# Audio-WestlakeU/FullSubNet

Measured on AMD Instinct MI355X. Metric: frames/sec (16 kHz, 512-FFT, hop 256), whole job, higher is better.
Workload: dtype f32

## Files before the change

### fullsubnet_amd/csrc/lstm_rec_x_kernels.hip

```cpp
#include "fsn_common.h"
#include "lstm_cell.h"

namespace {

__device__ __forceinline__ void lds_dma_fragment(const float* g, unsigned lds_base) {
    unsigned saved;
    asm volatile(
        "s_mov_b32 %0, m0\n\t"
        "s_mov_b32 m0, %1\n\t"
        "s_nop 0\n\t"
        "global_load_lds_dwordx4 %2, off\n\t"
        "s_nop 0\n\t"
        "s_mov_b32 m0, %0"
        : "=&s"(saved)
        : "s"(lds_base), "v"(g)
        : "memory");
}

__device__ __forceinline__ void lds_dma_fragment_s(const float* sbase, unsigned lane_bytes, unsigned lds_base) {
    unsigned saved;
    asm volatile(
        "s_mov_b32 %0, m0\n\t"
        "s_mov_b32 m0, %1\n\t"
        "s_nop 0\n\t"
        "global_load_lds_dwordx4 %2, %3\n\t"
        "s_nop 0\n\t"
        "s_mov_b32 m0, %0"
        : "=&s"(saved)
        : "s"(lds_base), "v"(lane_bytes), "s"(sbase)
        : "memory");
}

#ifndef FSN_REC_VCAP
#define FSN_REC_VCAP 76
#endif
template <int H, int RT, int UG, bool GRU, bool HSEQ>
__global__ __launch_bounds__((H / (16 * UG)) * 64) __attribute__((amdgpu_num_vgpr(FSN_REC_VCAP))) void lstm_rec_x_kernel(const float* __restrict__ xseq,
                                                                          const float* __restrict__ w_p,
                                                                          unsigned whh_off,
                                                                          const float* __restrict__ bias, int Tp,
                                                                          int Npad, const FsnRecFc fc) {
    constexpr int NW = H / (16 * UG);
    constexpr int KC = H / 16;
    constexpr int HS = H + 4;
    constexpr int ROWS = RT * 16;
    constexpr int SK = 6;
    constexpr int NSL = KC / SK;
    constexpr int NF = RT * SK;
    static_assert(KC % SK == 0 && SK % 2 == 0 && KC % 2 == 0, "slice width must divide the K range; chunks go in pairs");
    extern __shared__ __attribute__((aligned(16))) float xs[];
    float* hl = xs + 2 * NF * 256;
    float* wl = hl + ROWS * HS;

    const int lane = threadIdx.x & 63, wave = __builtin_amdgcn_readfirstlane(threadIdx.x >> 6);
    const int lr = lane & 15, lq = lane >> 4;
    const long n0 = (long)blockIdx.x * ROWS;
    if (!HSEQ)
        for (int i = threadIdx.x; i < 2 * H; i += NW * 64) {
            const int c = i / H, k = i % H;
            wl[i] = fc.w_p[(((k >> 4) * 64) + ((k & 15) >> 2) * 16 + c) * 4 + (k & 3)];
        }
    int fc_b0 = 0, fc_f0 = 0;
    float fc_bias0 = 0.f, fc_bias1 = 0.f;
    if (!HSEQ) {
        const long ng0 = n0 + fc.row0;
        fc_b0 = (int)(ng0 / fc.F);
        fc_f0 = (int)(ng0 - (long)fc_b0 * fc.F);
        fc_bias0 = fc.bias[0];
        fc_bias1 = fc.bias[1];
    }
    static_assert(RT >= 2 && RT <= 4, "two base registers reach row tiles 0-1 / 2-3");
    static_assert(!GRU || NSL % 2 == 0, "the GRU form skips whole passes of the x ring: slices per pass must be even");
    f32x4 cst[RT][UG], tmp[RT][UG];
#pragma unroll
    for (int rt = 0; rt < RT; ++rt)
#pragma unroll
        for (int u = 0; u < UG; ++u)
#pragma unroll
            for (int i = 0; i < 4; ++i) cst[rt][u][i] = 0.f;
    for (int i = threadIdx.x; i < ROWS * HS; i += NW * 64) hl[i] = 0.f;

    const unsigned xlane = (unsigned)(lr * H + 4 * lq);
    const unsigned xs_lds = (unsigned)(size_t)(__attribute__((address_space(3))) float*)xs;
    auto fill = [&](int buf, int t, int sl) {
        const float* src = xseq + ((long)t * Npad + n0) * H + sl * (SK * 16);
        for (int f = wave; f < NF; f += NW) {
            const int rt = f / SK, kcl = f - rt * SK;
            lds_dma_fragment(src + (rt * 16 * H + kcl * 16) + xlane,
                             __builtin_amdgcn_readfirstlane(xs_lds + (unsigned)((buf * NF + f) * 1024)));
        }
    };
    constexpr int FPW = (NF + NW - 1) / NW;
    int fsa_src[FPW], fsa_lds[FPW];
#pragma unroll
    for (int i = 0; i < FPW; ++i) {
        const int f = wave + i * NW, rt = f / SK, kcl = f - rt * SK;
        fsa_src[i] = __builtin_amdgcn_readfirstlane(rt * 16 * H + kcl * 16);
        fsa_lds[i] = __builtin_amdgcn_readfirstlane((int)xs_lds + f * 1024);
    }
    const unsigned xlane_bytes = xlane * 4u;
    auto fill_s = [&](int buf, int t, int sl) {
        const float* src = xseq + ((long)t * Npad + n0) * H + sl * (SK * 16);
#pragma unroll
        for (int i = 0; i < FPW; ++i)
            if (NF % NW == 0 || wave + i * NW < NF)
                lds_dma_fragment_s(src + fsa_src[i], xlane_bytes, (unsigned)(fsa_lds[i] + buf * (NF * 1024)));
    };
    fill(0, 0, 0);
    asm volatile("s_waitcnt vmcnt(0)" ::: "memory");
    __syncthreads();

    f32x4 b0[UG], b1[UG];
    const __amdgpu_buffer_rsrc_t wrsrc =
        __builtin_amdgcn_make_buffer_rsrc(const_cast<float*>(w_p), 0, 0x7fffffff, 0x00020000);
    const unsigned lane16 = (unsigned)lane * 16u;
    auto wofs = [&](int g, int u) { return (unsigned)((g * KC + wave * UG + u) * KC) * 256u; };
    auto wload = [&](unsigned ofs) {
        return __builtin_bit_cast(f32x4, __builtin_amdgcn_raw_buffer_load_b128(wrsrc, lane16, ofs * 4u, 0));
    };
    float bias_n[UG];
    {
        int g0 = 1;
        asm volatile("" : "+s"(g0));
#pragma unroll
        for (int u = 0; u < UG; ++u) {
            b0[u] = wload(wofs(g0, u));
            bias_n[u] = bias[(g0 * KC + wave * UG + u) * 16 + lr];
        }
    }
    auto mma = [&](f32x4 (&acc)[RT][UG], const float* a, int a_rt_stride, const f32x4 (&b)[UG]) {
#pragma unroll
        for (int rt = 0; rt < RT; ++rt) {
            const f32x4 av = *reinterpret_cast<const f32x4*>(a + rt * a_rt_stride);
#pragma unroll
            for (int jj = 0; jj < 4; ++jj)
#pragma unroll
                for (int u = 0; u < UG; ++u) acc[rt][u] = mfma16(av[jj], b[u][jj], acc[rt][u]);
        }
    };

    auto mma_fill = [&](f32x4 (&acc)[RT][UG], const float* a, int a_rt_stride, const f32x4 (&b)[UG], int buf, int nt, int nsl) {
        const f32x4 a0 = *reinterpret_cast<const f32x4*>(a), a1 = *reinterpret_cast<const f32x4*>(a + a_rt_stride);
#pragma unroll
        for (int jj = 0; jj < 4; ++jj)
#pragma unroll
            for (int u = 0; u < UG; ++u) acc[0][u] = mfma16(a0[jj], b[u][jj], acc[0][u]);
        __builtin_amdgcn_sched_barrier(0);
        if (nt < Tp) fill_s(buf, nt, nsl);
        __builtin_amdgcn_sched_barrier(0);
#pragma unroll
        for (int rt = 1; rt < RT; ++rt) {
            const f32x4 av = rt == 1 ? a1 : *reinterpret_cast<const f32x4*>(a + rt * a_rt_stride);
#pragma unroll
            for (int jj = 0; jj < 4; ++jj)
#pragma unroll
                for (int u = 0; u < UG; ++u) acc[rt][u] = mfma16(av[jj], b[u][jj], acc[rt][u]);
        }
    };

    for (int t = 0; t < Tp; ++t) {
#pragma unroll
        for (int pass = 0; pass < 4; ++pass) {
            __builtin_amdgcn_sched_barrier(0);
            int g = pass == 0 ? 1 : (pass == 1 ? 0 : pass);
            int gn = pass == 0 ? 0 : (pass == 1 ? 2 : (pass == 2 ? 3 : 1));
            asm volatile("" : "+s"(g));
            asm volatile("" : "+s"(gn));
            const bool hpart = t > 0 && !(GRU && pass == 2);
            const bool xpart = !(GRU && pass == 1 && t > 0);
            const bool prev_h = t > 0 && !(GRU && pass == 3);
            f32x4 acc[RT][UG];
            unsigned wx[UG], wh[UG], wxn[UG];
#pragma unroll
            for (int u = 0; u < UG; ++u) {
                wx[u] = wofs(g, u);
                wh[u] = wx[u] + whh_off;
                wxn[u] = wofs(gn, u) + ((GRU && pass == 0 && t > 0) ? whh_off : 0u);
                const float b = bias_n[u];
#pragma unroll
                for (int rt = 0; rt < RT; ++rt) acc[rt][u] = f32x4{b, b, b, b};
                bias_n[u] = bias[(gn * KC + wave * UG + u) * 16 + lr];
            }
#pragma unroll 1
            for (int sl = 0; sl < (xpart ? NSL : 0); ++sl) {
                const int j = pass * NSL + sl;
                if (j > 0 && !(sl == 0 && prev_h)) {
                    asm volatile("s_waitcnt vmcnt(%0)" ::"n"(UG) : "memory");
                    __builtin_amdgcn_fence(__ATOMIC_RELEASE, "workgroup", "local");
                    __builtin_amdgcn_s_barrier();
                    __builtin_amdgcn_fence(__ATOMIC_ACQUIRE, "workgroup", "local");
                }
                const int nsl = sl + 1 < NSL ? sl + 1 : 0;
                const int nt = (sl + 1 < NSL || pass < 3) ? t : t + 1;
                const float* xa = xs + ((j & 1) * NF) * 256 + lane * 4;
#pragma unroll
                for (int kk = 0; kk < SK; kk += 2) {
                    const int kc = sl * SK + kk;
#pragma unroll
                    for (int u = 0; u < UG; ++u)
                        b1[u] = wload(wx[u] + (unsigned)(kc + 1) * 256u);
                    __builtin_amdgcn_sched_barrier(0);
                    if (kk == 0) mma_fill(acc, xa, SK * 256, b0, (j + 1) & 1, nt, nsl);
                    else mma(acc, xa + kk * 256, SK * 256, b0);
                    __builtin_amdgcn_sched_barrier(0);
                    const bool more_x = kc + 2 < KC;
#pragma unroll
                    for (int u = 0; u < UG; ++u) {
                        b0[u] = wload(more_x ? wx[u] + (unsigned)(kc + 2) * 256u : (hpart ? wh[u] : wxn[u]));
                    }
                    __builtin_amdgcn_sched_barrier(0);
                    mma(acc, xa + (kk + 1) * 256, SK * 256, b1);
                    __builtin_amdgcn_sched_barrier(0);
                }
            }
            if (hpart) {
                typedef const __attribute__((address_space(3))) float* lds_cptr;
                unsigned hb01 = (unsigned)(size_t)(lds_cptr)(hl + lr * HS + 4 * lq), hb23 = hb01 + 32u * HS * 4u;
                asm volatile("" : "+v"(hb01));
                asm volatile("" : "+v"(hb23));
                lds_cptr ha01 = (lds_cptr)(size_t)hb01;
                lds_cptr ha23 = (lds_cptr)(size_t)hb23;
                auto mmah = [&](int kofs, const f32x4 (&b)[UG]) {
#pragma unroll
                    for (int rt = 0; rt < RT; ++rt) {
                        const f32x4 av = *reinterpret_cast<const __attribute__((address_space(3))) f32x4*>((rt < 2 ? ha01 : ha23) + (rt & 1) * 16 * HS + kofs);
#pragma unroll
                        for (int jj = 0; jj < 4; ++jj)
#pragma unroll
                            for (int u = 0; u < UG; ++u) acc[rt][u] = mfma16(av[jj], b[u][jj], acc[rt][u]);
                    }
                };
#pragma unroll 1
                for (int hs = 0; hs < NSL; ++hs) {
                    if (pass < 3 && hs == NSL / 2) {
                        asm volatile("s_waitcnt vmcnt(%0)" ::"n"(UG) : "memory");
                        __builtin_amdgcn_fence(__ATOMIC_RELEASE, "workgroup", "local");
                        __builtin_amdgcn_s_barrier();
                        __builtin_amdgcn_fence(__ATOMIC_ACQUIRE, "workgroup", "local");
                    }
#pragma unroll
                    for (int kk = 0; kk < SK; kk += 2) {
                        const int kc = hs * SK + kk;
#pragma unroll
                        for (int u = 0; u < UG; ++u) b1[u] = wload(wh[u] + (unsigned)(kc + 1) * 256u);
                        __builtin_amdgcn_sched_barrier(0);
                        mmah(kk * 16, b0);
                        __builtin_amdgcn_sched_barrier(0);
                        const bool more_h = kc + 2 < KC;
#pragma unroll
                        for (int u = 0; u < UG; ++u) b0[u] = wload(more_h ? wh[u] + (unsigned)(kc + 2) * 256u : wxn[u]);
                        __builtin_amdgcn_sched_barrier(0);
                        mmah((kk + 1) * 16, b1);
                        __builtin_amdgcn_sched_barrier(0);
                    }
                    ha01 += SK * 16;
                    ha23 += SK * 16;
                }
            }
#define FSN_REC_EPILOGUE2(VAR, EXPR)                                                                  \
    _Pragma("unroll") for (int rt = 0; rt < RT; ++rt)                                                 \
    _Pragma("unroll") for (int u = 0; u < UG; ++u) {                                                  \
        const f32x4 A = acc[rt][u], C = cst[rt][u], M = tmp[rt][u];                                   \
        (void)A, (void)C, (void)M;                                                                    \
        auto half = [&](f32x2 a, f32x2 c, f32x2 m) { (void)a, (void)c, (void)m; return EXPR; };       \
        VAR[rt][u] = cat2(half(lo2(A), lo2(C), lo2(M)), half(hi2(A), hi2(C), hi2(M)));                \
        asm volatile("" : "+v"(VAR[rt][u]));                                                          \
    }
            if constexpr (GRU) {
                if (pass == 0) {
                    FSN_REC_EPILOGUE2(tmp, sigmoid_fast2(a))
                } else if (pass == 1) {
                    FSN_REC_EPILOGUE2(tmp, m * a)
                } else if (pass == 2) {
                    FSN_REC_EPILOGUE2(tmp, tanh_fast2(a + m))
                } else {
                    FSN_REC_EPILOGUE2(cst, m + sigmoid_fast2(a) * (c - m))
                }
            } else if (pass == 0) {
                FSN_REC_EPILOGUE2(cst, sigmoid_fast2(a) * c)
            } else if (pass == 1) {
                FSN_REC_EPILOGUE2(tmp, sigmoid_fast2(a))
            } else if (pass == 2) {
                FSN_REC_EPILOGUE2(cst, c + m * tanh_fast2(a))
            } else {
                FSN_REC_EPILOGUE2(tmp, sigmoid_fast2(a) * tanh_fast2(c))
            }
#undef FSN_REC_EPILOGUE2
            __builtin_amdgcn_sched_barrier(0);
        }
        __builtin_amdgcn_fence(__ATOMIC_RELEASE, "workgroup", "local");
        __builtin_amdgcn_s_barrier();
        __builtin_amdgcn_fence(__ATOMIC_ACQUIRE, "workgroup", "local");
        {
            unsigned hwb = (unsigned)((4 * lq) * HS + (wave * UG) * 16 + lr);
            asm volatile("" : "+v"(hwb));
            float* hw = hl + hwb;
#pragma unroll
            for (int rt = 0; rt < RT; ++rt)
#pragma unroll
                for (int u = 0; u < UG; ++u)
#pragma unroll
                    for (int i = 0; i < 4; ++i) hw[(rt * 16 + i) * HS + u * 16] = GRU ? cst[rt][u][i] : tmp[rt][u][i];
        }
        __builtin_amdgcn_fence(__ATOMIC_RELEASE, "workgroup", "local");
        __builtin_amdgcn_s_barrier();
        __builtin_amdgcn_fence(__ATOMIC_ACQUIRE, "workgroup", "local");
        if (HSEQ) {
            float* dst = fc.crm_r + ((long)t * Npad + n0) * H;
            for (int i = threadIdx.x; i < ROWS * (H / 4); i += NW * 64) {
                const int row = i / (H / 4), c4 = i % (H / 4);
                *reinterpret_cast<f32x4*>(dst + (long)row * H + c4 * 4) =
                    *reinterpret_cast<const f32x4*>(hl + row * HS + c4 * 4);
            }
        } else {
            const int tid = threadIdx.x;
            if (tid < ROWS * 8) {
                const int part = tid & 3, c = (tid >> 2) & 1, row = tid >> 3;
                const float* hp = hl + row * HS + part * (H / 4);
                const float* wp = wl + c * H + part * (H / 4);
                float a0 = 0.f, a1 = 0.f;
#pragma unroll 2
                for (int k = 0; k < H / 4; k += 8) {
                    const f32x4 h0 = *reinterpret_cast<const f32x4*>(hp + k), w0 = *reinterpret_cast<const f32x4*>(wp + k);
                    const f32x4 h1 = *reinterpret_cast<const f32x4*>(hp + k + 4),
                                w1 = *reinterpret_cast<const f32x4*>(wp + k + 4);
                    a0 = fmaf(h0[0], w0[0], a0);
                    a0 = fmaf(h0[1], w0[1], a0);
                    a0 = fmaf(h0[2], w0[2], a0);
                    a0 = fmaf(h0[3], w0[3], a0);
                    asm volatile("" : "+v"(a0));
                    a1 = fmaf(h1[0], w1[0], a1);
                    a1 = fmaf(h1[1], w1[1], a1);
                    a1 = fmaf(h1[2], w1[2], a1);
                    a1 = fmaf(h1[3], w1[3], a1);
                }
                float v = a0 + a1;
                v += __builtin_bit_cast(float, __builtin_amdgcn_mov_dpp(__builtin_bit_cast(int, v), 0xB1, 0xF, 0xF, true));
                v += __builtin_bit_cast(float, __builtin_amdgcn_mov_dpp(__builtin_bit_cast(int, v), 0x4E, 0xF, 0xF, true));
                if (part == 0 && t >= fc.la && (int)n0 + row < fc.N) {
                    int f = fc_f0 + row, b = fc_b0;
                    while (f >= fc.F) {
                        f -= fc.F;
                        ++b;
                    }
                    (c ? fc.crm_i : fc.crm_r)[((long)b * fc.T + (t - fc.la)) * fc.FP + f] = v + (c ? fc_bias1 : fc_bias0);
                }
            }
        }
    }
}

template <int H, int RT, bool HSEQ, int CELL = 0, int UG = 2>
int launch_rec_x(const float* xseq, const float* wih_p, const float* whh_p, const float* bias, int Tp, int Npad,
                 int main_wgs, hipStream_t s, const FsnRecFc* fc, float* hseq_out) {
    constexpr int NW = H / (16 * UG);
    const size_t lds = ((size_t)RT * 16 * (H + 4) + 2 * H + (size_t)2 * RT * 6 * 256) * sizeof(float);
    auto kern = lstm_rec_x_kernel<H, RT, UG, CELL != 0, HSEQ>;
    if (lds > 160 * 1024 ||
        hipFuncSetAttribute(reinterpret_cast<const void*>(kern), hipFuncAttributeMaxDynamicSharedMemorySize,
                            (int)lds) != hipSuccess) {
        fsn_set_error("lstm_rec_x: cannot reserve %zu bytes of LDS", lds);
        return FSN_ERR_LAUNCH;
    }
    if (whh_p < wih_p || whh_p - wih_p > 0x3fffffffL) {
        fsn_set_error("lstm_rec_x: W_hh must follow W_ih in one packed buffer");
        return FSN_ERR_ARG;
    }
    FsnRecFc a{};
    if (fc) a = *fc;
    if (HSEQ) a.crm_r = hseq_out;
    hipLaunchKernelGGL(kern, dim3((unsigned)main_wgs), dim3(NW * 64), lds, s, xseq, wih_p, (unsigned)(whh_p - wih_p), bias,
                       Tp, Npad, a);
    return fsn_check_launch("lstm_rec_x_kernel");
}

}

bool fsn_lstm_rec_x_supported(int H, int RT) { return H == 384 && RT >= 2 && RT <= 4; }

int fsn_launch_lstm_rec_x(const float* xseq, const float* wih_p, const float* whh_p, const float* bias, int Tp, int Npad,
                          int H, int RT, int main_wgs, hipStream_t s, const FsnRecFc* fc, float* hseq_out, int cell) {
    if (((!fc || !fc->w_p) && !hseq_out) || !fsn_lstm_rec_x_supported(H, RT)) {
        fsn_set_error("lstm_rec_x: needs the fused output layer or a hidden-sequence buffer, H = 384 and 2 - 4 row tiles "
                      "(got H %d, RT %d)", H, RT);
        return FSN_ERR_ARG;
    }
    if (cell) {
        if (hseq_out) {
            if (RT == 2) return launch_rec_x<384, 2, true, 1>(xseq, wih_p, whh_p, bias, Tp, Npad, main_wgs, s, nullptr, hseq_out);
            if (RT == 3) return launch_rec_x<384, 3, true, 1>(xseq, wih_p, whh_p, bias, Tp, Npad, main_wgs, s, nullptr, hseq_out);
            return launch_rec_x<384, 4, true, 1>(xseq, wih_p, whh_p, bias, Tp, Npad, main_wgs, s, nullptr, hseq_out);
        }
        fsn_set_error("lstm_rec_x: the GRU cell is instantiated for the hidden-sequence form (its output layer is a separate launch)");
        return FSN_ERR_ARG;
    }
    if (hseq_out) {
        if (RT == 2) return launch_rec_x<384, 2, true>(xseq, wih_p, whh_p, bias, Tp, Npad, main_wgs, s, nullptr, hseq_out);
        if (RT == 3) return launch_rec_x<384, 3, true>(xseq, wih_p, whh_p, bias, Tp, Npad, main_wgs, s, nullptr, hseq_out);
        return launch_rec_x<384, 4, true>(xseq, wih_p, whh_p, bias, Tp, Npad, main_wgs, s, nullptr, hseq_out);
    }
    if (RT == 2) return launch_rec_x<384, 2, false>(xseq, wih_p, whh_p, bias, Tp, Npad, main_wgs, s, fc, nullptr);
    if (RT == 3) return launch_rec_x<384, 3, false>(xseq, wih_p, whh_p, bias, Tp, Npad, main_wgs, s, fc, nullptr);
    return launch_rec_x<384, 4, false>(xseq, wih_p, whh_p, bias, Tp, Npad, main_wgs, s, fc, nullptr);
}
```

Baseline: 147,900.

## Fuse LSTM input and cell gates into one paired pass per step

For the LSTM path, the recurrent kernel now computes the input gate and the candidate gate in a single pass, using two accumulator sets that share each LDS A-fragment read and each slice barrier. Each timestep goes from four gate passes to three, cutting x-ring barriers and A-operand reloads, and the tmp round-trip for the input gate is dropped. The cost is doubled accumulator and weight-register pressure in the paired pass, which may spill or lower occupancy. The unused non-scalar LDS DMA fill helper is removed and the initial fill uses the scalar-base variant.

```diff
diff --git a/fullsubnet_amd/csrc/lstm_rec_x_kernels.hip b/fullsubnet_amd/csrc/lstm_rec_x_kernels.hip
--- a/fullsubnet_amd/csrc/lstm_rec_x_kernels.hip
+++ b/fullsubnet_amd/csrc/lstm_rec_x_kernels.hip
@@ -2,20 +2,6 @@
 #include "lstm_cell.h"
 
 namespace {
-
-__device__ __forceinline__ void lds_dma_fragment(const float* g, unsigned lds_base) {
-    unsigned saved;
-    asm volatile(
-        "s_mov_b32 %0, m0\n\t"
-        "s_mov_b32 m0, %1\n\t"
-        "s_nop 0\n\t"
-        "global_load_lds_dwordx4 %2, off\n\t"
-        "s_nop 0\n\t"
-        "s_mov_b32 m0, %0"
-        : "=&s"(saved)
-        : "s"(lds_base), "v"(g)
-        : "memory");
-}
 
 __device__ __forceinline__ void lds_dma_fragment_s(const float* sbase, unsigned lane_bytes, unsigned lds_base) {
     unsigned saved;
@@ -82,14 +68,6 @@
 
     const unsigned xlane = (unsigned)(lr * H + 4 * lq);
     const unsigned xs_lds = (unsigned)(size_t)(__attribute__((address_space(3))) float*)xs;
-    auto fill = [&](int buf, int t, int sl) {
-        const float* src = xseq + ((long)t * Npad + n0) * H + sl * (SK * 16);
-        for (int f = wave; f < NF; f += NW) {
-            const int rt = f / SK, kcl = f - rt * SK;
-            lds_dma_fragment(src + (rt * 16 * H + kcl * 16) + xlane,
-                             __builtin_amdgcn_readfirstlane(xs_lds + (unsigned)((buf * NF + f) * 1024)));
-        }
-    };
     constexpr int FPW = (NF + NW - 1) / NW;
     int fsa_src[FPW], fsa_lds[FPW];
 #pragma unroll
@@ -106,7 +84,7 @@
             if (NF % NW == 0 || wave + i * NW < NF)
                 lds_dma_fragment_s(src + fsa_src[i], xlane_bytes, (unsigned)(fsa_lds[i] + buf * (NF * 1024)));
     };
-    fill(0, 0, 0);
+    fill_s(0, 0, 0);
     asm volatile("s_waitcnt vmcnt(0)" ::: "memory");
     __syncthreads();
 
@@ -118,24 +96,28 @@
     auto wload = [&](unsigned ofs) {
         return __builtin_bit_cast(f32x4, __builtin_amdgcn_raw_buffer_load_b128(wrsrc, lane16, ofs * 4u, 0));
     };
-    float bias_n[UG];
+    float bias_n[GRU ? 1 : 2][UG];
     {
         int g0 = 1;
         asm volatile("" : "+s"(g0));
 #pragma unroll
         for (int u = 0; u < UG; ++u) {
             b0[u] = wload(wofs(g0, u));
-            bias_n[u] = bias[(g0 * KC + wave * UG + u) * 16 + lr];
-        }
-    }
-    auto mma = [&](f32x4 (&acc)[RT][UG], const float* a, int a_rt_stride, const f32x4 (&b)[UG]) {
+            bias_n[0][u] = bias[(g0 * KC + wave * UG + u) * 16 + lr];
+        }
+    }
+    auto mma = [&](f32x4 (&acc)[RT][UG], const float* a, int a_rt_stride, const f32x4 (&b)[UG], bool pairwise = false) {
 #pragma unroll
         for (int rt = 0; rt < RT; ++rt) {
+            if (pairwise && rt == 2) __builtin_amdgcn_sched_barrier(0);
             const f32x4 av = *reinterpret_cast<const f32x4*>(a + rt * a_rt_stride);
 #pragma unroll
             for (int jj = 0; jj < 4; ++jj)
 #pragma unroll
                 for (int u = 0; u < UG; ++u) acc[rt][u] = mfma16(av[jj], b[u][jj], acc[rt][u]);
+            if (pairwise)
+#pragma unroll
+                for (int u = 0; u < UG; ++u) asm volatile("" : "+v"(acc[rt][u]));
         }
     };
 
@@ -158,59 +140,107 @@
         }
     };
 
+    constexpr int NP = GRU ? 4 : 3;
+    constexpr int NGM = GRU ? 1 : 2;
+    static_assert((NP * NSL) % 2 == 0, "slices per step must be even: the ring stage of slice j is j & 1 in every step");
+    auto gates_of = [](int pass) { return !GRU && pass == 1 ? 2 : 1; };
+    auto gate_of = [](int pass, int q) {
+        if (GRU) return pass == 0 ? 1 : (pass == 1 ? 0 : pass);
+        return pass == 0 ? 1 : (pass == 1 ? (q ? 2 : 0) : 3);
+    };
+    auto slice_barrier = [&](bool pair) {
+        if (pair) asm volatile("s_waitcnt vmcnt(%0)" ::"n"(2 * UG) : "memory");
+        else asm volatile("s_waitcnt vmcnt(%0)" ::"n"(UG) : "memory");
+        __builtin_amdgcn_fence(__ATOMIC_RELEASE, "workgroup", "local");
+        __builtin_amdgcn_s_barrier();
+        __builtin_amdgcn_fence(__ATOMIC_ACQUIRE, "workgroup", "local");
+    };
     for (int t = 0; t < Tp; ++t) {
 #pragma unroll
-        for (int pass = 0; pass < 4; ++pass) {
+        for (int pass = 0; pass < NP; ++pass) {
             __builtin_amdgcn_sched_barrier(0);
-            int g = pass == 0 ? 1 : (pass == 1 ? 0 : pass);
-            int gn = pass == 0 ? 0 : (pass == 1 ? 2 : (pass == 2 ? 3 : 1));
-            asm volatile("" : "+s"(g));
-            asm volatile("" : "+s"(gn));
+            const int pn = pass + 1 < NP ? pass + 1 : 0;
+            const bool pair = gates_of(pass) == 2;
             const bool hpart = t > 0 && !(GRU && pass == 2);
             const bool xpart = !(GRU && pass == 1 && t > 0);
             const bool prev_h = t > 0 && !(GRU && pass == 3);
-            f32x4 acc[RT][UG];
-            unsigned wx[UG], wh[UG], wxn[UG];
-#pragma unroll
-            for (int u = 0; u < UG; ++u) {
-                wx[u] = wofs(g, u);
-                wh[u] = wx[u] + whh_off;
-                wxn[u] = wofs(gn, u) + ((GRU && pass == 0 && t > 0) ? whh_off : 0u);
-                const float b = bias_n[u];
-#pragma unroll
-                for (int rt = 0; rt < RT; ++rt) acc[rt][u] = f32x4{b, b, b, b};
-                bias_n[u] = bias[(gn * KC + wave * UG + u) * 16 + lr];
+            f32x4 acc[NGM][RT][UG];
+            unsigned wx[NGM][UG], wh[NGM][UG], wxn[UG];
+#pragma unroll
+            for (int q = 0; q < NGM; ++q) {
+                if (q >= gates_of(pass)) continue;
+                int g = gate_of(pass, q);
+                asm volatile("" : "+s"(g));
+#pragma unroll
+                for (int u = 0; u < UG; ++u) {
+                    wx[q][u] = wofs(g, u);
+                    wh[q][u] = wx[q][u] + whh_off;
+                    const float b = bias_n[q][u];
+#pragma unroll
+                    for (int rt = 0; rt < RT; ++rt) acc[q][rt][u] = f32x4{b, b, b, b};
+                }
+            }
+#pragma unroll
+            for (int q = 0; q < NGM; ++q) {
+                if (q >= gates_of(pn)) continue;
+                int gn = gate_of(pn, q);
+                asm volatile("" : "+s"(gn));
+#pragma unroll
+                for (int u = 0; u < UG; ++u) {
+                    if (q == 0) wxn[u] = wofs(gn, u) + ((GRU && pass == 0 && t > 0) ? whh_off : 0u);
+                    bias_n[q][u] = bias[(gn * KC + wave * UG + u) * 16 + lr];
+                }
+            }
+            if (pair) {
+#pragma unroll
+                for (int u = 0; u < UG; ++u) b1[u] = wload(wx[NGM - 1][u]);
             }
 #pragma unroll 1
             for (int sl = 0; sl < (xpart ? NSL : 0); ++sl) {
                 const int j = pass * NSL + sl;
-                if (j > 0 && !(sl == 0 && prev_h)) {
-                    asm volatile("s_waitcnt vmcnt(%0)" ::"n"(UG) : "memory");
-                    __builtin_amdgcn_fence(__ATOMIC_RELEASE, "workgroup", "local");
-                    __builtin_amdgcn_s_barrier();
-                    __builtin_amdgcn_fence(__ATOMIC_ACQUIRE, "workgroup", "local");
-                }
+                if (j > 0 && !(sl == 0 && prev_h)) slice_barrier(pair);
                 const int nsl = sl + 1 < NSL ? sl + 1 : 0;
-                const int nt = (sl + 1 < NSL || pass < 3) ? t : t + 1;
+                const int nt = (sl + 1 < NSL || pass < NP - 1) ? t : t + 1;
                 const float* xa = xs + ((j & 1) * NF) * 256 + lane * 4;
-#pragma unroll
-                for (int kk = 0; kk < SK; kk += 2) {
-                    const int kc = sl * SK + kk;
-#pragma unroll
-                    for (int u = 0; u < UG; ++u)
-                        b1[u] = wload(wx[u] + (unsigned)(kc + 1) * 256u);
-                    __builtin_amdgcn_sched_barrier(0);
-                    if (kk == 0) mma_fill(acc, xa, SK * 256, b0, (j + 1) & 1, nt, nsl);
-                    else mma(acc, xa + kk * 256, SK * 256, b0);
-                    __builtin_amdgcn_sched_barrier(0);
-                    const bool more_x = kc + 2 < KC;
-#pragma unroll
-                    for (int u = 0; u < UG; ++u) {
-                        b0[u] = wload(more_x ? wx[u] + (unsigned)(kc + 2) * 256u : (hpart ? wh[u] : wxn[u]));
+                if (pair) {
+#pragma unroll
+                    for (int kk = 0; kk < SK; ++kk) {
+                        const int kc = sl * SK + kk;
+                        const bool more_x = kc + 1 < KC;
+                        if (kk == 0) mma_fill(acc[0], xa, SK * 256, b0, (j + 1) & 1, nt, nsl);
+                        else mma(acc[0], xa + kk * 256, SK * 256, b0, true);
+                        __builtin_amdgcn_sched_barrier(0);
+#pragma unroll
+                        for (int u = 0; u < UG; ++u)
+                            b0[u] = wload(more_x ? wx[0][u] + (unsigned)(kc + 1) * 256u : (hpart ? wh[0][u] : wxn[u]));
+                        __builtin_amdgcn_sched_barrier(0);
+                        mma(acc[NGM - 1], xa + kk * 256, SK * 256, b1, true);
+                        __builtin_amdgcn_sched_barrier(0);
+#pragma unroll
+                        for (int u = 0; u < UG; ++u)
+                            b1[u] = wload(more_x ? wx[NGM - 1][u] + (unsigned)(kc + 1) * 256u : wh[NGM - 1][u]);
+                        __builtin_amdgcn_sched_barrier(0);
                     }
-                    __builtin_amdgcn_sched_barrier(0);
-                    mma(acc, xa + (kk + 1) * 256, SK * 256, b1);
-                    __builtin_amdgcn_sched_barrier(0);
+                } else {
+#pragma unroll
+                    for (int kk = 0; kk < SK; kk += 2) {
+                        const int kc = sl * SK + kk;
+#pragma unroll
+                        for (int u = 0; u < UG; ++u)
+                            b1[u] = wload(wx[0][u] + (unsigned)(kc + 1) * 256u);
+                        __builtin_amdgcn_sched_barrier(0);
+                        if (kk == 0) mma_fill(acc[0], xa, SK * 256, b0, (j + 1) & 1, nt, nsl);
+                        else mma(acc[0], xa + kk * 256, SK * 256, b0);
+                        __builtin_amdgcn_sched_barrier(0);
+                        const bool more_x = kc + 2 < KC;
+#pragma unroll
+                        for (int u = 0; u < UG; ++u) {
+                            b0[u] = wload(more_x ? wx[0][u] + (unsigned)(kc + 2) * 256u : (hpart ? wh[0][u] : wxn[u]));
+                        }
+                        __builtin_amdgcn_sched_barrier(0);
+                        mma(acc[0], xa + (kk + 1) * 256, SK * 256, b1);
+                        __builtin_amdgcn_sched_barrier(0);
+                    }
                 }
             }
             if (hpart) {
@@ -220,38 +250,56 @@
                 asm volatile("" : "+v"(hb23));
                 lds_cptr ha01 = (lds_cptr)(size_t)hb01;
                 lds_cptr ha23 = (lds_cptr)(size_t)hb23;
-                auto mmah = [&](int kofs, const f32x4 (&b)[UG]) {
+                auto mmah = [&](f32x4 (&acc)[RT][UG], int kofs, const f32x4 (&b)[UG], bool pairwise = false) {
 #pragma unroll
                     for (int rt = 0; rt < RT; ++rt) {
+                        if (pairwise && rt == 2) __builtin_amdgcn_sched_barrier(0);
                         const f32x4 av = *reinterpret_cast<const __attribute__((address_space(3))) f32x4*>((rt < 2 ? ha01 : ha23) + (rt & 1) * 16 * HS + kofs);
 #pragma unroll
                         for (int jj = 0; jj < 4; ++jj)
 #pragma unroll
                             for (int u = 0; u < UG; ++u) acc[rt][u] = mfma16(av[jj], b[u][jj], acc[rt][u]);
+                        if (pairwise)
+#pragma unroll
+                            for (int u = 0; u < UG; ++u) asm volatile("" : "+v"(acc[rt][u]));
                     }
                 };
 #pragma unroll 1
                 for (int hs = 0; hs < NSL; ++hs) {
-                    if (pass < 3 && hs == NSL / 2) {
-                        asm volatile("s_waitcnt vmcnt(%0)" ::"n"(UG) : "memory");
-                        __builtin_amdgcn_fence(__ATOMIC_RELEASE, "workgroup", "local");
-                        __builtin_amdgcn_s_barrier();
-                        __builtin_amdgcn_fence(__ATOMIC_ACQUIRE, "workgroup", "local");
-                    }
-#pragma unroll
-                    for (int kk = 0; kk < SK; kk += 2) {
-                        const int kc = hs * SK + kk;
-#pragma unroll
-                        for (int u = 0; u < UG; ++u) b1[u] = wload(wh[u] + (unsigned)(kc + 1) * 256u);
-                        __builtin_amdgcn_sched_barrier(0);
-                        mmah(kk * 16, b0);
-                        __builtin_amdgcn_sched_barrier(0);
-                        const bool more_h = kc + 2 < KC;
-#pragma unroll
-                        for (int u = 0; u < UG; ++u) b0[u] = wload(more_h ? wh[u] + (unsigned)(kc + 2) * 256u : wxn[u]);
-                        __builtin_amdgcn_sched_barrier(0);
-                        mmah((kk + 1) * 16, b1);
-                        __builtin_amdgcn_sched_barrier(0);
+                    if (pass < NP - 1 && hs == NSL / 2) slice_barrier(pair);
+                    if (pair) {
+#pragma unroll
+                        for (int kk = 0; kk < SK; ++kk) {
+                            const int kc = hs * SK + kk;
+                            const bool more_h = kc + 1 < KC;
+                            mmah(acc[0], kk * 16, b0, true);
+                            __builtin_amdgcn_sched_barrier(0);
+#pragma unroll
+                            for (int u = 0; u < UG; ++u) b0[u] = wload(more_h ? wh[0][u] + (unsigned)(kc + 1) * 256u : wxn[u]);
+                            __builtin_amdgcn_sched_barrier(0);
+                            mmah(acc[NGM - 1], kk * 16, b1, true);
+                            __builtin_amdgcn_sched_barrier(0);
+#pragma unroll
+                            for (int u = 0; u < UG; ++u)
+                                b1[u] = wload(more_h ? wh[NGM - 1][u] + (unsigned)(kc + 1) * 256u : wxn[u]);
+                            __builtin_amdgcn_sched_barrier(0);
+                        }
+                    } else {
+#pragma unroll
+                        for (int kk = 0; kk < SK; kk += 2) {
+                            const int kc = hs * SK + kk;
+#pragma unroll
+                            for (int u = 0; u < UG; ++u) b1[u] = wload(wh[0][u] + (unsigned)(kc + 1) * 256u);
+                            __builtin_amdgcn_sched_barrier(0);
+                            mmah(acc[0], kk * 16, b0);
+                            __builtin_amdgcn_sched_barrier(0);
+                            const bool more_h = kc + 2 < KC;
+#pragma unroll
+                            for (int u = 0; u < UG; ++u) b0[u] = wload(more_h ? wh[0][u] + (unsigned)(kc + 2) * 256u : wxn[u]);
+                            __builtin_amdgcn_sched_barrier(0);
+                            mmah(acc[0], (kk + 1) * 16, b1);
+                            __builtin_amdgcn_sched_barrier(0);
+                        }
                     }
                     ha01 += SK * 16;
                     ha23 += SK * 16;
@@ -260,10 +308,10 @@
 #define FSN_REC_EPILOGUE2(VAR, EXPR)                                                                  \
     _Pragma("unroll") for (int rt = 0; rt < RT; ++rt)                                                 \
     _Pragma("unroll") for (int u = 0; u < UG; ++u) {                                                  \
-        const f32x4 A = acc[rt][u], C = cst[rt][u], M = tmp[rt][u];                                   \
-        (void)A, (void)C, (void)M;                                                                    \
-        auto half = [&](f32x2 a, f32x2 c, f32x2 m) { (void)a, (void)c, (void)m; return EXPR; };       \
-        VAR[rt][u] = cat2(half(lo2(A), lo2(C), lo2(M)), half(hi2(A), hi2(C), hi2(M)));                \
+        const f32x4 A = acc[0][rt][u], A2 = acc[NGM - 1][rt][u], C = cst[rt][u], M = tmp[rt][u];      \
+        (void)A, (void)A2, (void)C, (void)M;                                                          \
+        auto half = [&](f32x2 a, f32x2 a2, f32x2 c, f32x2 m) { (void)a, (void)a2, (void)c, (void)m; return EXPR; }; \
+        VAR[rt][u] = cat2(half(lo2(A), lo2(A2), lo2(C), lo2(M)), half(hi2(A), hi2(A2), hi2(C), hi2(M))); \
         asm volatile("" : "+v"(VAR[rt][u]));                                                          \
     }
             if constexpr (GRU) {
@@ -279,9 +327,7 @@
             } else if (pass == 0) {
                 FSN_REC_EPILOGUE2(cst, sigmoid_fast2(a) * c)
             } else if (pass == 1) {
-                FSN_REC_EPILOGUE2(tmp, sigmoid_fast2(a))
-            } else if (pass == 2) {
-                FSN_REC_EPILOGUE2(cst, c + m * tanh_fast2(a))
+                FSN_REC_EPILOGUE2(cst, c + sigmoid_fast2(a) * tanh_fast2(a2))
             } else {
                 FSN_REC_EPILOGUE2(tmp, sigmoid_fast2(a) * tanh_fast2(c))
             }
```

New measurement: 141,400. 0.956x the previous value.
